# HIITMetagenomics/dsm-framework

Hardware: AMD Instinct MI355X
Metric: enumerated substrings/sec (Emax=2.0) (higher is better)
Workload: dtype u32

## Files before the change

### dsm-framework_amd/csrc/engine.hip

```cpp
#include <sched.h>

#include <algorithm>
#include <atomic>
#include <chrono>
#include <cmath>
#include <condition_variable>
#include <cstdlib>
#include <cstring>
#include <deque>
#include <map>
#include <functional>
#include <memory>
#include <mutex>
#include <sstream>
#include <thread>
#include <type_traits>

#include "common.h"
#include "scan.h"
#include "setorder.h"
#include "stream_parse.h"
#include "lfstep.h"
#include "entropy_tables.h"
#include "textemit.h"
// ... 134 lines not shown
        for (u32 l = 0; l < x.nlocal; ++l) {
            const u32 m = pb[(u64)l * x.F + u];
#pragma unroll
            for (int c = 0; c < 4; ++c) nT4[c] += (m >> c) & 1u;
        }
    }
}

template <typename P>
__global__ __launch_bounds__(256) void advance_reduce_kernel(Xchg x, u16* __restrict__ sinfo, u64* __restrict__ kplane, u32* __restrict__ cnt4, u32 nbp) {
    __shared__ u32 wtot[4][4];
    const u32 u = blockIdx.x * TILE + threadIdx.x;
    const int lane = threadIdx.x & 63, w = threadIdx.x >> 6;
    u32 nT4[4] = {0, 0, 0, 0};
    if (u < x.F) {
        parent_eval<P>(x, u, nT4);
        uint2 q;
        q.x = nT4[0] | (nT4[1] << 16);
        q.y = nT4[2] | (nT4[3] << 16);
        *reinterpret_cast<uint2*>(sinfo + (size_t)u * 4) = q;
    }
    u64 bal[4];
#pragma unroll
    for (int c = 0; c < 4; ++c) bal[c] = __ballot(nT4[c] != 0);
    if (lane < 4) {
        const u64 b = DSM_PICK(bal, lane);
        wtot[w][lane] = (u32)__popcll(b);
        kplane[((size_t)blockIdx.x * 4 + w) * 4 + lane] = b;
    }
    __syncthreads();
    if (threadIdx.x < 4) cnt4[(size_t)threadIdx.x * nbp + blockIdx.x] = wtot[0][threadIdx.x] + wtot[1][threadIdx.x] + wtot[2][threadIdx.x] + wtot[3][threadIdx.x];
}

struct FilterArgs {
    u32 F;
    u32 depth;
    u32 d;
    u32 pmin, pmax, mindepth;
    double emin, emax;
    u32 exact_order;
};

constexpr double ENT_MARGIN = 1e-4;

template <typename P>
__device__ __forceinline__ bool filter_node(const FilterArgs& a, const Xchg& x, u32 v, u32 t, u32 nc, u32 same) {
    if (a.depth < a.mindepth) return false;
    if (a.pmax != 0 && t > a.pmax) return false;
    if (t < a.pmin) return false;
    if (nc == 1 && same) return false;
    u64 sumN = a.d;
    double s = 0;
    u32 l = 0xFF;
    if (x_is_nm8(x)) {
        u32 w[8];
        x_words8(x, v, w);
#pragma unroll
        for (int g = 0; g < 8; ++g) {
            const u64 f = w[g] & (PACK_FMAX - 1);
            if (f) {
                const u32 lg = w[g] >> 13;
                l = l == 0xFF ? lg : (l == lg ? l : 5u);
                sumN += f;
                if (a.emax > 0) s += (double)(f + 1) * (double)__log2f((float)(f + 1));
            }
        }
    } else {
        for (u32 g = 0; g < a.d; ++g) {
            u64 f = (u64)x_freq<P>(x, g, v);
            if (f) {
                u32 lg = x_pl<P>(x, g, v) >> 4;
                l = l == 0xFF ? lg : (l == lg ? l : 5u);
                sumN += f;
                if (a.emax > 0) s += (double)(f + 1) * (double)__log2f((float)(f + 1));
            }
        }
    }
    if (l >= 1 && l <= 4) return false;
    if (a.emax > 0) {
        double e = (double)__log2f((float)sumN) - s / (double)sumN;
        if (e < a.emin - ENT_MARGIN || e > a.emax + ENT_MARGIN) return false;
    }
    return true;
}

constexpr u32 PW_CHUNK = 16;
constexpr u32 SREC_FIRST = 4u, SREC_LAST = 8u;
__device__ __forceinline__ uint2 child_path_word(const uint2 parent, u32 u, u32 plevel, u32 c) {
    const u32 r = plevel & (PW_CHUNK - 1);
    return r == 0 ? make_uint2(u, c) : make_uint2(parent.x, parent.y | (c << (2 * r)));
}

struct AdvanceOut {
    u32* slot;
    uint2* sa;
    uint2* pw;
    const uint2* parent_pw;
    const u32* width;
    u32 pw_after_slot;
    u32 plevel;
    u32 kshift;
    u32 cand_copy;
    u16* nT;
    u8* samechild;
    const u16* parent_nT;
    const u64* kplane;
    u64* kplane_w;
    u32* kcum;
    const u32* cnt4;
    u32* cnt_clear;
    u32 nbp;
    const u16* sinfo;
    u32 eval;
    u32 single;
    u32* const* rp;
    u32* rp0;
    const u64* const* splane;
    u32 rp_index;
    const u32* const* tpos;
    u32 nlocal, rank;
    u32 seg;
    u32 cap;
    u32* h_totals;
    u32 filter_on;
    FilterArgs fa;
    u64* candbits;
    u64* wsum;
    uint4* crec;
    u32 crec_cap;
};

struct PublishArgs {
    const u32* total;
    const u64* cand;
    const u8* cmax_base;
    u64 cmax_bpr;
    u32 cmax_world;
    u32* clear;
    u32* next;
    uint4* packet;
    u32 seq;
    uint4* bc_header;
    const u32* grand;
};
__global__ void publish_kernel(PublishArgs a) {
    __shared__ u32 wide;
    if (threadIdx.x == 0) wide = 0;
    __syncthreads();
    for (u32 r = threadIdx.x; r < a.cmax_world; r += blockDim.x) {
        const u64 m = *reinterpret_cast<const u64*>(a.cmax_base + (u64)r * a.cmax_bpr);
        if (m >= PACK_FMAX) atomicOr(&wide, m >= 65535 ? 3u : 2u);
    }
    const u32 tot = threadIdx.x == 0 ? *a.total : 0u;
    u64 cand = threadIdx.x == 0 && a.cand ? *a.cand : 0ull;
    if (threadIdx.x == 0 && a.grand) { const u64 c = (u64)(*a.grand - tot); cand = c | (c << 32); }
    __syncthreads();
    if (a.clear && threadIdx.x < 4) a.clear[threadIdx.x] = 0;
    if (threadIdx.x == 0) {
        if (a.next) { a.next[0] = tot; a.next[1] = wide; }
        const uint4 pk = make_uint4(a.seq, tot | ((wide & 1u) << 31) | ((wide >> 1) << 30), (u32)cand, (u32)(cand >> 32));
        if (a.bc_header) *a.bc_header = make_uint4(BC_OK, pk.y, 0u, 0u);
        *a.packet = pk;
    }
}

template <typename P>
// ... 97 lines not shown
        }
    }
    if (threadIdx.x == 0) o.h_totals[0] = total;
}

template <typename P>
__global__ __launch_bounds__(256) void advance_wave_kernel(Xchg x, AdvanceOut o) {
    __shared__ u32 wcnt[4][4];
    const u32 F = (u32)x.F;
    const int lane = threadIdx.x & 63;
    const u32 nw = (F + 63) >> 6;
    const u32 tile = xcd_block();
    const u32 wi = (u32)__builtin_amdgcn_readfirstlane((int)(threadIdx.x >> 6));
    const u32 w = tile * 4 + wi;
    const bool wave_in = w < nw;
    const u32 wc = wave_in ? w : 0u;
    const u64 lt = (1ull << lane) - 1;
    const u32 u = w * 64 + lane;
    const bool in = wave_in && u < F;
    const u32 uc = in ? u : 0u;
    u64 up[4];
    u32 base[4];
#pragma unroll
    for (int c = 0; c < 4; ++c) {
        up[c] = o.kplane[((size_t)wc << o.kshift) + c];
        base[c] = o.cnt4[(size_t)c * o.nbp + tile];
    }
    uint2 mypw = make_uint2(0u, 0u);
    uint2* pw = o.pw;
    u32 width = 0;
    if (o.pw_after_slot) width = o.width[0];
    if (pw) mypw = o.parent_pw[uc];
    uint2 sq = make_uint2(0u, 0u);
    if (o.sinfo) sq = *reinterpret_cast<const uint2*>(o.sinfo + (size_t)uc * 4);
    u32 myT = 1u;
    if (!o.single) myT = (u32)o.parent_nT[uc];
    u64 candw = 0;
    if (o.cand_copy && (lane == 4 || lane == 5)) candw = o.kplane[((size_t)wc << 3) + lane];
    u64 f1 = 0;
    u32 l1 = 0;
    if (o.single && o.filter_on) { f1 = (u64)x_freq<P>(x, 0, uc); l1 = x_pl<P>(x, 0, uc) >> 4; }
    if (!wave_in) {
#pragma unroll
        for (int c = 0; c < 4; ++c) up[c] = 0;
    }
    if (lane < 4) wcnt[wi][lane] = (u32)__popcll(DSM_PICK(up, lane));
    __syncthreads();
    if (!wave_in) return;
    if (o.pw_after_slot) pw = reinterpret_cast<uint2*>(reinterpret_cast<u8*>(o.slot) + (((size_t)width * 4 + 255) & ~(size_t)255));
    u32 cum[4];
#pragma unroll
    for (int c = 0; c < 4; ++c) {
        u32 before = 0;
#pragma unroll
        for (u32 q = 0; q < 3; ++q) before += q < wi ? wcnt[q][c] : 0u;
        cum[c] = base[c] + before;
    }
    u32 nT4[4] = {0, 0, 0, 0};
    if (o.sinfo) {
        if (in) { nT4[0] = sq.x & 0xFFFFu; nT4[1] = sq.x >> 16; nT4[2] = sq.y & 0xFFFFu; nT4[3] = sq.y >> 16; }
    } else {
#pragma unroll
        for (int c = 0; c < 4; ++c) nT4[c] = (u32)((up[c] >> lane) & 1);
    }
    if (lane < 4) {
        o.kcum[(size_t)w * 4 + lane] = DSM_PICK(cum, lane);
        if (o.kplane_w) o.kplane_w[(size_t)w * 4 + lane] = DSM_PICK(up, lane);
        if (o.cnt_clear && wi == 0) o.cnt_clear[(size_t)lane * o.nbp + tile] = 0;
    }
    if (o.cand_copy) {
        if (lane == 4) o.candbits[w] = candw;
        if (lane == 5) o.wsum[w] = candw;
    }
    u32 pres = 0, lastT = 0, vj[4];
#pragma unroll
    for (int c = 0; c < 4; ++c) {
        vj[c] = cum[c] + (u32)__popcll(up[c] & lt);
        if (nT4[c]) { pres |= 1u << c; lastT = nT4[c]; }
    }
    const u32 nc = __popc(pres);
    if (!in) myT = 0;
    const u32 same = o.single ? 1u : ((nc == 1 && lastT == myT) ? 1u : 0u);
    if (o.filter_on) {
        bool cand;
        if (o.single) {
            const FilterArgs& a = o.fa;
            cand = in && a.depth >= a.mindepth && 1u >= a.pmin && nc != 1 && !(f1 != 0 && l1 >= 1 && l1 <= 4);
            if (cand && a.emax > 0) {
                const u64 sumN = 1ull + f1;
                const double sl = f1 ? (double)(f1 + 1) * (double)__log2f((float)(f1 + 1)) : 0.0;
                const double e = (double)__log2f((float)sumN) - sl / (double)sumN;
                if (e < a.emin - ENT_MARGIN || e > a.emax + ENT_MARGIN) cand = false;
            }
        } else {
            cand = in && filter_node<P>(o.fa, x, u, myT, nc, same);
        }
        const u64 bits = __ballot(cand);
        u64 pairs = (u64)__popcll(bits);
        if (!o.single) pairs = wave_sum_u64(cand ? (u64)myT : 0ull);
        if (lane == 0) { o.candbits[w] = bits; o.wsum[w] = (u64)__popcll(bits) | (pairs << 32); }
    }
    if (!in) return;
    if (!o.single) o.samechild[u] = (u8)same;
#pragma unroll
    for (int c = 0; c < 4; ++c) {
        if (((pres >> c) & 1u) && vj[c] < o.cap) {
            if (o.slot) o.slot[vj[c]] = 4u * u + (u32)c;
            if (pw) pw[vj[c]] = child_path_word(mypw, u, o.plevel, (u32)c);
            if (o.sa) o.sa[vj[c]] = make_uint2(u, (u32)c | ((pres & ((1u << c) - 1u)) ? 0u : SREC_FIRST) | ((pres >> (c + 1)) ? 0u : SREC_LAST));
            if (!o.single) o.nT[vj[c]] = (u16)nT4[c];
        }
    }
    if (o.single) {
#pragma unroll
        for (int c = 0; c < 4; ++c)
            if (((pres >> c) & 1u) && vj[c] < o.cap) o.rp0[vj[c]] = (u32)c * o.seg + w * 64u + (u32)__popcll(up[c] & lt);
        return;
    }
    for (u32 sl = 0; sl < o.nlocal && pres && (o.tpos || o.rp_index); ++sl) {
        u32* rp = o.rp[sl];
        if (o.tpos) {
            const u32 m = x_pl<P>(x, o.rank * o.nlocal + sl, u) & 15u;
            const u32 h = m ? o.tpos[sl][u] : 0u;
#pragma unroll
            for (int c = 0; c < 4; ++c)
                if (((pres >> c) & 1u) && vj[c] < o.cap) rp[vj[c]] = ((m >> c) & 1u) ? h + (u32)__popc(m & ((1u << c) - 1u)) : DEAD;
        } else {
            const u64* sp = o.splane[sl] + (size_t)w * 4;
#pragma unroll
            for (int c = 0; c < 4; ++c) {
                if (!((pres >> c) & 1u) || vj[c] >= o.cap) continue;
                const u64 mine = sp[c];
                rp[vj[c]] = ((mine >> lane) & 1) ? (u32)c * o.seg + w * 64u + (u32)__popcll(mine & lt) : DEAD;
            }
        }
    }
}

template <typename P>
__global__ __launch_bounds__(256) void advance_single_kernel(Xchg x, AdvanceOut o) {
    const int lane = threadIdx.x & 63;
    const u32 F = (u32)x.F;
    const u32 nw = (F + 63) >> 6;
    const u32 tile = (u32)__builtin_amdgcn_readfirstlane((int)(xcd_block() * 4 + (threadIdx.x >> 6)));
    if (tile >= o.nbp) return;
    const u64 lt = (1ull << lane) - 1;
    const u64* __restrict__ line = o.kplane + (size_t)tile * 32;
    uint2 mypw[4];
#pragma unroll
    for (int q = 0; q < 4; ++q) {
        const u32 u = (tile * 4 + (u32)q) * 64 + lane;
        mypw[q] = o.parent_pw[u < F ? u : 0u];
    }
    u64 copyw = 0;
    if (lane < 32) copyw = line[lane];
    u32 cum[4];
#pragma unroll
    for (int c = 0; c < 4; ++c) cum[c] = o.cnt4[(size_t)c * o.nbp + tile];
    u64 up[4][4];
#pragma unroll
    for (int q = 0; q < 4; ++q)
#pragma unroll
        for (int c = 0; c < 4; ++c) up[q][c] = tile * 4 + (u32)q < nw ? line[q * 8 + c] : 0ull;
    {
        const u32 q = (u32)lane >> 3, j = (u32)lane & 7u, w = tile * 4 + q;
        if (lane < 32 && w < nw) {
            if (j < 4) o.kplane_w[(size_t)w * 4 + j] = copyw;
            else if (o.cand_copy && j == 4) o.candbits[w] = copyw;
            else if (o.cand_copy && j == 5) o.wsum[w] = copyw;
        }
    }
    const u32 r = o.plevel & (PW_CHUNK - 1);
    u32 kc = 0;
    u32 cbase = 0;
    u64 cbq[4] = {0, 0, 0, 0};
    u32 ncq[4] = {0, 0, 0, 0};
    u64 fq[4] = {0, 0, 0, 0};
    if (o.crec) {
        cbase = o.cnt4[(size_t)4 * o.nbp + tile] - o.cnt4[(size_t)4 * o.nbp];
#pragma unroll
        for (int q = 0; q < 4; ++q) {
            if (tile * 4 + (u32)q < nw) { cbq[q] = line[q * 8 + 4]; ncq[q] = (u32)line[q * 8 + 5]; }
            const u32 u = (tile * 4 + (u32)q) * 64 + lane;
            if ((cbq[q] >> lane) & 1ull) fq[q] = (u64)x_freq<P>(x, 0, u);
        }
    }
#pragma unroll
    for (int q = 0; q < 4; ++q) {
        const u32 w = tile * 4 + (u32)q, u = w * 64 + lane;
        const uint2 ppw = mypw[q];
        if (o.crec && cbq[q]) {
            const u32 k = cbase + bits_below_lane(cbq[q]);
            if (((cbq[q] >> lane) & 1ull) && k < o.crec_cap) o.crec[k] = make_uint4(u, 0u, (u32)fq[q], (u32)(fq[q] >> 32));
        }
        cbase += ncq[q];
#pragma unroll
        for (int c = 0; c < 4; ++c) {
            const u64 m = up[q][c];
            if (lane == q * 4 + c) kc = cum[c];
            const u32 below = bits_below_lane(m);
            const u32 vj = cum[c] + below;
            if (((m >> lane) & 1ull) && vj < o.cap) {
                o.rp0[vj] = (u32)c * o.seg + w * 64u + below;
                o.pw[vj] = r == 0 ? make_uint2(u, (u32)c) : make_uint2(ppw.x, ppw.y | ((u32)c << (2 * r)));
            }
            cum[c] += (u32)__popcll(m);
        }
    }
    if (lane < 16 && tile * 4 + ((u32)lane >> 2) < nw) o.kcum[(size_t)tile * 16 + lane] = kc;
}

__global__ __launch_bounds__(256) void lite_count_kernel(const u64* __restrict__ kplane, u32 nw, u32* __restrict__ cnt4, u32 nbp, u32 kshift, u32 cand_row = 0) {
    const u32 tile = blockIdx.x * 64 + (threadIdx.x >> 2), c = threadIdx.x & 3;
    if (tile >= nbp) return;
    u32 s = 0, nc = 0;
    if (cand_row && tile * 4 + c < nw) nc = (u32)kplane[((size_t)(tile * 4 + c) << 3) + 5];
#pragma unroll
    for (u32 q = 0; q < 4; ++q) {
        const u32 w = tile * 4 + q;
        if (w < nw) s += (u32)__popcll(kplane[((size_t)w << kshift) + c]);
    }
    cnt4[(size_t)c * nbp + tile] = s;
    if (cand_row) {
        nc += __shfl_xor(nc, 1, 64);
        nc += __shfl_xor(nc, 2, 64);
        if (c == 0) cnt4[(size_t)4 * nbp + tile] = nc;
    }
}
__global__ __launch_bounds__(256) void lite_slot_kernel(const u64* __restrict__ kplane, u32 F, const u32* __restrict__ cnt4, u32 nbp, u32 single_tile,
                                                        u32* __restrict__ slot, u32 cap) {
    const int lane = threadIdx.x & 63;
    const u32 nw = (F + 63) >> 6;
    const u32 tile = xcd_block();
    const u32 wi = threadIdx.x >> 6, w = tile * 4 + wi;
    if (w >= nw) return;
    const u32 u = w * 64 + lane;
    u32 base = 0;
#pragma unroll
    for (int c = 0; c < 4; ++c) {
        u32 before = 0, all = 0;
#pragma unroll
        for (u32 q = 0; q < 4; ++q) {
            const u32 wq = tile * 4 + q;
            const u32 t = wq < nw ? (u32)__popcll(kplane[(size_t)wq * 4 + c]) : 0u;
            before += q < wi ? t : 0u;
            all += t;
        }
        const u64 up = kplane[(size_t)w * 4 + c];
        const u32 first = (single_tile ? base : cnt4[(size_t)c * nbp + tile]) + before;
        base += all;
        const u32 vj = first + (u32)__popcll(up & ((1ull << lane) - 1));
        if (u < F && ((up >> lane) & 1) && vj < cap) slot[vj] = 4u * u + (u32)c;
    }
}

template <typename P>
__global__ __launch_bounds__(256) void order_kernel(u32 F, Xchg x, const u16* __restrict__ nT, const u64* __restrict__ order, Kids kids,
                                                    u64* __restrict__ order_next) {
    __shared__ u32 qn;
    __shared__ u32 qu[256];
    __shared__ u64 qm[256], qo[256];
    if (threadIdx.x == 0) qn = 0;
    __syncthreads();
    const u32 u = blockIdx.x * blockDim.x + threadIdx.x;
    if (u < F) {
        const u32 cnt = nT[u];
        const u64 ord = order[u];
        u64 mbyid = 0;
        u32 um = 0;
        if (x_is_nm8(x)) {
            u32 w[8];
            x_words8(x, u, w);
#pragma unroll
            for (int g = 0; g < 8; ++g) { const u32 m = (w[g] >> 9) & 15u; mbyid |= (u64)m << (4 * g); um |= m; }
        } else {
            for (u32 k = 0; k < cnt; ++k) {
                const u32 r = (u32)((ord >> (4 * k)) & 15);
                const u32 m = x_pl<P>(x, r, u) & 15u;
                mbyid |= (u64)m << (4 * r);
                um |= m;
            }
        }
        if (um && !(um & (um - 1))) {
            u64 rev = 0;
            for (u32 k = 0; k < cnt; ++k) {
                const u32 r = (u32)((ord >> (4 * k)) & 15);
                if ((mbyid >> (4 * r)) & 15) rev = (rev << 4) | r;
            }
            order_next[kid_index(kids, u, (u32)(__ffs((int)um) - 1))] = rev;
        } else if (um) {
            const u32 q = atomicAdd(&qn, 1u);
            qu[q] = u; qm[q] = mbyid; qo[q] = ord;
// ... 1474 lines not shown
        x.nm = node_major(w9) ? 1u : 0u;
        return x;
    }

    int alloc_kids(LevelHost& lv) {
        const size_t nw = ((size_t)lv.n + TILE - 1) / TILE * 4;
        ARENA_GET(lv.kplane, u64, 4 * nw);
        ARENA_GET(lv.kcum, u32, 4 * nw);
        return 0;
    }

    hipEvent_t pool_event(size_t k) {
        while (evpool.size() <= k) {
            hipEvent_t e = nullptr;
            if (hipEventCreateWithFlags(&e, hipEventDisableSystemFence) != hipSuccess) return nullptr;
            evpool.push_back(e);
        }
        return evpool[k];
    }

    struct BcastGuard {
        Engine* e;
        size_t gather_bytes = 0;
        void* gather_into = nullptr;
        size_t bytes = 0;
        explicit BcastGuard(Engine* e_) : e(e_) {}
        void arm(size_t b) { gather_bytes = 0; bytes = b; }
        void arm_next(size_t g, void* into, size_t b) { gather_bytes = g; gather_into = into; bytes = b; }
        void disarm() { gather_bytes = 0; bytes = 0; }
        ~BcastGuard() {
            if (!bytes) return;
            if (gather_bytes) (void)e->prm.gather(e->prm.owner_ctx, e->owner, e->xsend, gather_into, gather_bytes, (void*)e->st);
            const u32 hdr[4] = {BC_ABORT, 0, 0, 0};
            if (hipMemcpyAsync(e->bc_buf, hdr, 16, hipMemcpyHostToDevice, e->st) == hipSuccess) (void)hipStreamSynchronize(e->st);
            (void)e->prm.bcast(e->prm.owner_ctx, e->owner, e->bc_buf, bytes, (void*)e->st);
        }
    };

    u32 col_bytes(bool w16, bool w9) const { return w9 ? 2u : (w16 ? 3u : (u32)sizeof(P) + 1); }
    u64 level_bytes(u32 F, bool w16, bool w9) const { return (((u64)nlocal * F * col_bytes(w16, w9) + 15) & ~15ull) + 16; }
    static size_t bcast_bytes(u32 F) { return 16 + (size_t)((F + 63) >> 6) * 32; }
    u32 level_cap(bool w16) const { return w16 ? Fcap : FcapW; }
    int check_width(u32 Fn, bool w16) {
        if (Fn > level_cap(w16)) return fail(DSM_E_CAPACITY, "frontier wider than the device buffers: use a longer prefix or a larger arena_bytes");
        return 0;
    }
    u32 decode_level(u32 word, bool* w16, bool* w9) const {
        *w16 = !(word >> 31) && !trie_mode;
        *w9 = *w16 && !((word >> 30) & 1u);
        return word & 0x3FFFFFFFu;
    }
    int upload_order(int k, const u16* ro, size_t n) {
        if (d <= 13) {
            u64 ord = 0;
            for (size_t i = 0; i < n; ++i) ord |= (u64)ro[i] << (4 * i);
            DSM_HIP(hipMemcpyAsync(order[k], &ord, sizeof(u64), hipMemcpyHostToDevice, st));
        } else {
            DSM_HIP(hipMemcpyAsync(order16[k], ro, n * sizeof(u16), hipMemcpyHostToDevice, st));
        }
        return 0;
    }

    struct Walk {
        std::string prefix;
        RunOpts o;
        std::vector<LevelHost> L;
        u32 order_mode = 0;
        bool emitting = false;
        bool emit_failed = false;
        bool trace = false;
        size_t nev = 0;
        u32 F = 1, depth = 0;
        bool w16 = false, w9 = false;
        BcastGuard owed;
        explicit Walk(Engine* e) : owed(e) {}
        int cur() const { return (int)(depth & 1); }
    };
    struct Sweep {
        Xchg x;
        size_t mark = 0;
        u32* slot = nullptr;
        bool filtered = false;
        u32 crec_cap = 0;
        u32 Fn = 0;
        bool w16 = false, w9 = false;
        bool spec_hit = false;
    };

    int run(const char* prefix_c, dsm_tuple_sink tsink, dsm_byte_sink bsink, void* ctx, const RunOpts& o = RunOpts()) {
        Walk w(this);
        w.prefix = prefix_c ? prefix_c : "";
        w.o = o;
        for (char ch : w.prefix)
            if (ch != 'A' && ch != 'C' && ch != 'G' && ch != 'T')
                return fail(DSM_E_INVAL, "prefix must be over A,C,G,T");
        DSM_HIP(hipSetDevice(device));
        for (int s_ = 0; s_ < nlocal && !trie_mode; ++s_)
            if (!idx[s_]->dev.blk) return fail(DSM_E_INVAL, "an index of this miner is offloaded: dsm_index_reload first");
        arena.off = 0;
        earena.off = 0;
        carena.off = 0;
        w.emitting = o.emit;
        w.L.reserve(512);
        DSM_HIP(hipMemsetAsync(d_counters, 0, (size_t)COUNTER_SHARDS * 8 * sizeof(u64), st));
        if (cntraw) DSM_HIP(hipMemsetAsync(cntraw, 0, (4 * (size_t)(Seg / TILE) + 8) * sizeof(u32), st));
        DSM_HIP(hipEventRecord(ev0, st));
        if (int rc = root_level(w)) return rc;
        w.order_mode = (d < 2 || prm.pmax == 1) ? 0u : (d <= 13 ? 1u : 2u);
        stats.pair_order_exact = 1;
        w.trace = getenv("DSM_TRACE_LEVELS") != nullptr;
        DSM_HIP(hipMemsetAsync(multi ? xsend : xrecv[0], 0, XHDR, st));
        if (int rc = launch_lf(w, 0, 1, w.w16, w.w9, w.L[0].slot)) return rc;
        while (true) {
            if (int rc = exchange(w)) return rc;
            if (owner_mode && !is_owner) {
                bool more = false;
                if (int rc = client_level(w, &more)) return rc;
                if (!more) break;
                continue;
            }
            if (owner_mode) { if (int rc = owner_precheck(w)) return rc; }
            Sweep s;
            LevelHost child;
            if (int rc = advance(w, s)) return rc;
            if (int rc = publish(w, s)) return rc;
            if (int rc = commit(w, s, child)) return rc;
            if (int rc = capture_level(w, s.Fn, child.slot, child.pw)) return rc;
            if (s.filtered) {
                int erc = emit_store(w.L[w.depth], w.F, w.depth, s.x, w.cur(), w.order_mode, s.crec_cap);
                if (erc == DSM_E_CAPACITY && multi) { w.emit_failed = true; w.emitting = false; }
                else if (erc) return erc;
            }
            DSM_HIP(hipGetLastError());
            if (pend.submit && (w.F >= 200000u || w.depth >= 24)) { if (int rc = flush_pending()) return rc; }
            count_level(w);
            if (!s.Fn) break;
            w.L.push_back(child);
            step(w, s.Fn, s.w16, s.w9);
            if (w.L.size() > 60000) return fail(DSM_E_CAPACITY, "trie deeper than 60000 levels");
        }
        timeline("levels done", w.prefix.c_str());
        if (int rc = flush_pending()) return rc;
        if (int rc = finish_prefix(w, tsink, bsink, ctx)) return rc;
        return read_back(w);
    }

    int root_level(Walk& w) {
        const char* bases = "ACGT";
        for (int s = 0; s < nlocal && trie_mode; ++s) {
            const u32 zero = 0;
            DSM_HIP(hipMemcpyAsync(rp[0][s], &zero, sizeof(u32), hipMemcpyHostToDevice, st));
            stats.reported += tries[s]->nodes;
        }
        for (int s = 0; s < nlocal && !trie_mode; ++s) {
            const IndexMeta& m = idx[s]->meta;
            P h[REC_FIELDS];
            for (int f = 0; f < REC_FIELDS; ++f) h[f] = 0;
            h[0] = 0;
            h[1] = (P)(m.n - 1);
            u8 hmask = 0;
            int slot = 0;
            for (int a = 0; a < 4; ++a) {
                u64 lo = m.C[(int)bases[a]], cnt = m.codes[(int)bases[a]].count;
                if (cnt) { h[2 + 2 * slot] = (P)lo; h[3 + 2 * slot] = (P)(lo + cnt - 1); ++slot; hmask |= (u8)(1u << a); }
            }
            for (int f = 0; f < REC_FIELDS; ++f)
                DSM_HIP(hipMemcpyAsync(rec[0][s] + (size_t)f * RcapW, &h[f], sizeof(P), hipMemcpyHostToDevice, st));
            DSM_HIP(hipMemcpyAsync(rec[0][s] + (size_t)REC_FIELDS * RcapW, &hmask, 1, hipMemcpyHostToDevice, st));
            const u32 zero = 0;
            DSM_HIP(hipMemcpyAsync(rp[0][s], &zero, sizeof(u32), hipMemcpyHostToDevice, st));
            if (self_mode) {
                const u64 one = 1;
                DSM_HIP(hipMemcpyAsync(splane2[s], &one, sizeof(u64), hipMemcpyHostToDevice, st));
            }
            stats.lf_steps += 8;
            for (int a = 0; a < 4; ++a) stats.rank_ops += 2 * m.lfcost[a];
        }
        LevelHost root;
        root.n = 1;
        ARENA_GET(root.slot, u32, 1);
        ARENA_GET(root.pw, uint2, 1);
        if (int rc = alloc_kids(root)) return rc;
        if (self_mode) DSM_HIP(hipMemsetAsync(root.slot, 0, sizeof(u32), st));
        DSM_HIP(hipMemsetAsync(root.pw, 0, sizeof(uint2), st));
        w.L.push_back(root);
        u16 rootT = (u16)d;
        DSM_HIP(hipMemcpyAsync(nT[0], &rootT, sizeof(u16), hipMemcpyHostToDevice, st));
        std::vector<u16> seq(d), ro(d + 1), tmp(so_work_size(d, d));
        for (u32 k = 0; k < d; ++k) seq[k] = (u16)k;
        set_iteration_order<u16>(seq.data(), d, ro.data(), tmp.data(), d);
        return upload_order(0, ro.data(), d);
    }

    int launch_lf(Walk& w, u32 depth, u32 F, bool w16, bool w9, const u32* lslot, u64 Fmax = 0) {
        const char* bases = "ACGT";
        const bool dynamic = Fmax != 0;
        const bool fmt_in = depth > 0 && w.w16 && !trie_mode;
        const int cur = (int)(depth & 1), nxt = cur ^ 1;
        const u32 colb = col_bytes(w16, w9), fb = colb - 1;
        u8* send = multi ? xsend : xrecv[cur];
        ExpandArgs ea;
        memset(&ea, 0, sizeof ea);
        ea.F = F; ea.nbp = (F + TILE - 1) / TILE; ea.fmin = prm.fmin; ea.w16 = w9 ? 2u : (w16 ? 1u : 0u);
        ea.seg = seg_of(w16 && !trie_mode); ea.cap = 4 * ea.seg;
        ea.seg_in = seg_of(fmt_in); ea.cap_in = 4 * ea.seg_in;
        const bool nm = node_major(w9);
        ea.cstride = nm ? (u32)nlocal : 1u;
        if (dynamic) {
            ea.dyn = d_dyn;
            ea.dyn_mask = 3u;
            ea.dyn_expect = (w16 ? 0u : 1u) | (w9 ? 0u : 2u);
            ea.fcap = level_cap(w16);
        }
        unsigned long long* d_childmax = reinterpret_cast<unsigned long long*>(send);
        if (depth < w.prefix.size()) {
            const char* q = strchr(bases, w.prefix[depth]);
            ea.allowed = 1u << (q - bases);
            ea.symbol_phase = 0;
// ... 131 lines not shown
        if (nbp > 1) {
            hipLaunchKernelGGL(lite_count_kernel, dim3((nbp + 63) / 64), dim3(256), 0, st, planes, nwv, cnt4, nbp, 2u);
            exclusive_scan<u32, u32>(cnt4, cnt4, (size_t)4 * nbp, scan_tmp, d_totals, st);
        }
        hipLaunchKernelGGL(lite_slot_kernel, dim3(nbp), dim3(256), 0, st, planes, F, cnt4, nbp, nbp == 1 ? 1u : 0u, lite_slot[nxt], Fcap);
        DSM_HIP(hipGetLastError());
        if (int rc = capture_level(w, Fn, lite_slot[nxt], nullptr)) return rc;
        if (int rc = launch_lf(w, w.depth + 1, Fn, w16, w9, lite_slot[nxt])) return rc;
        step(w, Fn, w16, w9);
        return 0;
    }

    int owner_precheck(Walk& w) {
        static const int test_owner_fail = getenv("DSM_TEST_OWNER_FAIL") ? atoi(getenv("DSM_TEST_OWNER_FAIL")) : -1;
        const size_t bc_bytes = bcast_bytes(w.F);
        w.owed.arm(bc_bytes);
        if (test_owner_fail >= 0 && (int)w.depth == test_owner_fail) return fail(DSM_E_SINK, "injected owner failure (DSM_TEST_OWNER_FAIL)");
        const size_t wc = (size_t)w.F * 4 < Fcap ? (size_t)w.F * 4 : Fcap;
        const size_t need = wc * 12 + 512 + ((wc + TILE - 1) / TILE * 4) * 48 + 4096;
        if (arena.off + need <= arena.cap) return 0;
        const u32 hdr[4] = {BC_CAPACITY, 0, 0, 0};
        DSM_HIP(hipMemcpyAsync(bc_buf, hdr, 16, hipMemcpyHostToDevice, st));
        DSM_HIP(hipStreamSynchronize(st));
        w.owed.disarm();
        if (prm.bcast(prm.owner_ctx, owner, bc_buf, bc_bytes, (void*)st)) return fail(DSM_E_SINK, "bcast callback failed");
        return fail(DSM_E_CAPACITY, "device arena exhausted: use a longer prefix or a larger arena_bytes");
    }

    int advance(Walk& w, Sweep& s) {
        const u32 F = w.F, depth = w.depth;
        const int cur = w.cur(), nxt = cur ^ 1;
        s.x = xview(cur, F, w.w16, w.w9);
        const Xchg& x = s.x;
        LevelHost& me = w.L[depth];
        if (stream_mode && depth >= 1) {
            ARENA_GET(me.srec, uint4, F);
            ARENA_GET(me.clen, u8, F);
            hipLaunchKernelGGL((keep_kernel<P>), grid_for(F), dim3(256), 0, st, F, x, sa[cur], me.srec, me.clen);
        }
        if (!stream_mode && w.emitting && depth >= 1 && depth >= w.o.emit_lo && depth <= w.o.emit_hi) {
            int erc = emit_alloc(me, F);
            if (erc == DSM_E_CAPACITY && multi) { w.emit_failed = true; w.emitting = false; }
            else if (erc) return erc;
            else s.filtered = true;
        }
        s.mark = arena.off;
        const bool keep_slot = self_mode, keep_pw = !stream_mode;
        const size_t wcap = (size_t)F * 4 < Fcap ? (size_t)F * 4 : Fcap;
        u8* window = arena.get<u8>(wcap * ((keep_slot ? 4 : 0) + (keep_pw ? 8 : 0)) + 512);
        if (!window) return fail(DSM_E_CAPACITY, "device arena exhausted: use a longer prefix or a larger arena_bytes");
        s.slot = keep_slot ? reinterpret_cast<u32*>(window) : nullptr;
        const u32 nbp = (F + TILE - 1) / TILE;
        AdvanceOut ao;
        memset(&ao, 0, sizeof ao);
        ao.slot = s.slot; ao.nT = nT[nxt]; ao.samechild = samechild;
        if (stream_mode) ao.sa = sa[nxt];
        if (keep_pw) {
            ao.pw = reinterpret_cast<uint2*>(window);
            ao.pw_after_slot = keep_slot ? 1u : 0u;
            ao.parent_pw = me.pw;
            ao.plevel = depth;
        }
        ao.parent_nT = nT[cur]; ao.nlocal = (u32)nlocal; ao.rank = (u32)rank;
        ao.cap = (u32)wcap;
        ao.seg = seg_of(w.w16 && !trie_mode);
        ao.h_totals = d_pub_tot;
        ao.rp = d_rp_tab[nxt];
        ao.rp0 = rp[nxt][0];
        ao.tpos = trie_mode ? d_tpos_tab : nullptr;
        ao.splane = d_splane_tab;
        ao.rp_index = self_mode ? 0u : 1u;
        ao.kcum = me.kcum; ao.cnt4 = cnt4; ao.nbp = nbp; ao.kshift = 2;
        ao.width = d_totals;
        const bool merged = d > 1 || trie_mode;
        if (merged && nbp == 1) {
            ao.eval = 1; ao.kplane_w = me.kplane;
        } else if (merged) {
            hipLaunchKernelGGL((advance_reduce_kernel<P>), dim3(nbp), dim3(256), 0, st, x, sinfo, me.kplane, cnt4, nbp);
            ao.kplane = me.kplane; ao.sinfo = sinfo;
        } else {
            ao.kplane = splane[0]; ao.kplane_w = me.kplane; ao.single = 1;
            ao.kshift = 3;
        }
        const bool lean = !merged && nbp > 1 && keep_pw && !keep_slot && !stream_mode;
        if (lean && s.filtered && carena.cap) {
            const size_t room = (carena.cap - carena.off) / sizeof(uint4);
            s.crec_cap = (u32)(room < (size_t)F ? room : (size_t)F);
        }
        const bool fold = s.crec_cap > 0;
        if (nbp > 1) {
            if (!merged) hipLaunchKernelGGL(lite_count_kernel, dim3((nbp + 63) / 64), dim3(256), 0, st, splane[0], (F + 63) >> 6, cntraw, nbp, 3u, fold ? 1u : 0u);
            exclusive_scan<u32, u32>(merged ? cnt4 : cntraw, cnt4, (size_t)(fold ? 5 : 4) * nbp, scan_tmp, d_totals, st);
        }
        const bool fused_filter = s.filtered && nbp > 1;
        if (fused_filter) {
            ao.fa = filter_args(F, depth, w.order_mode); ao.candbits = me.cand_bits; ao.wsum = cand_wsum;
            if (ao.single) ao.cand_copy = 1;
            else ao.filter_on = 1;
        }
        if (fold) { ao.crec = reinterpret_cast<uint4*>(carena.base + carena.off); ao.crec_cap = s.crec_cap; }
        if (nbp == 1) hipLaunchKernelGGL((advance_down_kernel<P>), dim3(1), dim3(256), 0, st, x, ao);
        else if (lean) hipLaunchKernelGGL((advance_single_kernel<P>), dim3((nbp + 3) / 4), dim3(256), 0, st, x, ao);
        else hipLaunchKernelGGL((advance_wave_kernel<P>), dim3(nbp), dim3(256), 0, st, x, ao);
        if (s.filtered) {
            if (int erc = emit_filter(me, F, depth, x, cur, w.order_mode, !fused_filter, fold)) return erc;
        }
        return 0;
    }

    int publish(Walk& w, Sweep& s) {
        const u32 F = w.F, nbp = (F + TILE - 1) / TILE;
        const int nxt = w.cur() ^ 1;
        PublishArgs pa;
        memset(&pa, 0, sizeof pa);
        pa.total = nbp == 1 ? d_pub_tot : d_totals;
        pa.cmax_base = s.x.base; pa.cmax_bpr = s.x.bpr; pa.cmax_world = (u32)world;
        if (s.filtered) pa.cand = d_totals64;
        if (s.crec_cap) {
            pa.total = cnt4 + (size_t)4 * nbp;
            pa.grand = d_totals;
            pa.cand = nullptr;
        }
        pa.clear = reinterpret_cast<u32*>(multi ? xsend : xrecv[nxt]);
        pa.packet = reinterpret_cast<uint4*>(h_totals + 304); pa.seq = ++pub_seq;
        pa.next = spec_mode ? d_dyn : nullptr;
        pa.bc_header = owner_mode ? reinterpret_cast<uint4*>(bc_buf) : nullptr;
        hipLaunchKernelGGL(publish_kernel, dim3(1), dim3(64), 0, st, pa);
        if (owner_mode) {
            const size_t bc_bytes = bcast_bytes(F);
            DSM_HIP(hipMemcpyAsync(bc_buf + 16, w.L[w.depth].kplane, bc_bytes - 16, hipMemcpyDeviceToDevice, st));
            w.owed.disarm();
            if (prm.bcast(prm.owner_ctx, owner, bc_buf, bc_bytes, (void*)st)) return fail(DSM_E_SINK, "bcast callback failed");
            stats.exchange_bytes_sent += bc_bytes * (u64)(world - 1);
        }
        if (spec_mode) { if (int rc = launch_lf(w, w.depth + 1, 0, w.w16, w.w9, s.slot, (u64)F * 4)) return rc; }
        u32 pk[4];
        if (int rc = wait_packet(pk)) return rc;
        s.Fn = decode_level(pk[1], &s.w16, &s.w9);
        s.spec_hit = spec_mode && s.Fn > 0 && s.Fn <= level_cap(s.w16) && s.w16 == w.w16 && s.w9 == w.w9;
        if (spec_mode && !s.spec_hit) --stats.expand_launches;
        h_totals[300] = pk[2]; h_totals[301] = pk[3];
        if (int rc = check_width(s.Fn, s.w16)) return rc;
        if (owner_mode) {
            if (!s.Fn) w.owed.arm(16);
            else w.owed.arm_next((size_t)level_bytes(s.Fn, s.w16, s.w9), xrecv[nxt], bcast_bytes(s.Fn));
        }
        return 0;
    }
    int wait_packet(u32 pk[4]) {
        volatile u32* fl = h_totals + 304;
        u32 spins = 0;
        while (*fl != pub_seq) {
            if ((++spins & 0xFFFFu) == 0 && hipStreamQuery(st) != hipErrorNotReady) {
                DSM_HIP(hipStreamSynchronize(st));
                if (*fl != pub_seq) return fail(DSM_E_HIP, "publish kernel did not report");
                break;
            }
            __builtin_ia32_pause();
        }
        std::atomic_thread_fence(std::memory_order_acquire);
        for (int q = 0; q < 4; ++q) pk[q] = fl[q];
        return 0;
    }

    int commit(Walk& w, const Sweep& s, LevelHost& child) {
        const u32 F = w.F, Fn = s.Fn;
        const int cur = w.cur(), nxt = cur ^ 1;
        arena.off = s.mark;
        child.n = Fn;
        if (!Fn) return 0;
        if (self_mode) child.slot = arena.get<u32>(Fn);
        if (!stream_mode) child.pw = arena.get<uint2>(Fn);
        if (int rc = alloc_kids(child)) return rc;
        if (s.spec_hit) {
            stats.expand_slots += Fn;
            stats.expand_column_bytes += (u64)Fn * col_bytes(s.w16, s.w9);
        } else {
            if (int rc = launch_lf(w, w.depth + 1, Fn, s.w16, s.w9, child.slot)) return rc;
        }
        const Kids kids = w.L[w.depth].kids();
        if (!(w.o.emit || w.o.capture)) {}
        else if (w.order_mode == 1)
            hipLaunchKernelGGL((order_kernel<P>), grid_for(F), dim3(256), 0, st, F, s.x, nT[cur], order[cur], kids, order[nxt]);
        else if (w.order_mode == 2 && d <= 64)
            hipLaunchKernelGGL((order_big_kernel<P, 64>), grid_for(F, 64), dim3(64), 0, st, F, s.x, nT[cur], order16[cur], kids, order16[nxt]);
        else if (w.order_mode == 2)
            hipLaunchKernelGGL((order_big_kernel<P, 273>), grid_for(F, 64), dim3(64), 0, st, F, s.x, nT[cur], order16[cur], kids, order16[nxt]);
        if (w.order_mode && w.o.seed && w.depth + 1 == w.o.seed->depth) {
            const std::vector<u16>& so = w.o.seed->ord[0];
            if (int rc = upload_order(nxt, so.data(), so.size())) return rc;
        }
        return 0;
    }

    int capture_level(Walk& w, u32 Fn, const u32* slot, const uint2* pw) {
        NodeOrder* cap = w.o.capture;
        if (!Fn || !cap || w.depth + 1 != cap->depth) return 0;
        const int nxt = w.cur() ^ 1;
        const bool client = owner_mode && !is_owner;
        std::vector<u32> hs(Fn);
        std::vector<u16> hn(Fn);
        if (slot) DSM_HIP(hipMemcpyAsync(hs.data(), slot, (size_t)Fn * sizeof(u32), hipMemcpyDeviceToHost, st));
        else if (stream_mode) {
            std::vector<uint2> hr(Fn);
            DSM_HIP(hipMemcpyAsync(hr.data(), sa[nxt], (size_t)Fn * sizeof(uint2), hipMemcpyDeviceToHost, st));
            DSM_HIP(hipStreamSynchronize(st));
            for (u32 v = 0; v < Fn; ++v) hs[v] = hr[v].y & 3u;
        } else {
            std::vector<uint2> hp(Fn);
            DSM_HIP(hipMemcpyAsync(hp.data(), pw, (size_t)Fn * sizeof(uint2), hipMemcpyDeviceToHost, st));
            DSM_HIP(hipStreamSynchronize(st));
            for (u32 v = 0; v < Fn; ++v) hs[v] = (hp[v].y >> (2 * (w.depth % PW_CHUNK))) & 3u;
        }
        if (!client) DSM_HIP(hipMemcpyAsync(hn.data(), nT[nxt], (size_t)Fn * sizeof(u16), hipMemcpyDeviceToHost, st));
        DSM_HIP(hipStreamSynchronize(st));
        const u32 order_mode = client ? 0u : w.order_mode;
        cap->sym.clear();
        cap->ord.clear();
        for (u32 v = 0; v < Fn; ++v) {
            cap->sym.push_back(hs[v] & 3);
            std::vector<u16> o(d == 1 || client ? 1 : hn[v]);
            if (order_mode == 1) {
                u64 ord = 0;
                DSM_HIP(hipMemcpy(&ord, order[nxt] + v, sizeof(u64), hipMemcpyDeviceToHost));
                for (u32 k = 0; k < hn[v]; ++k) o[k] = (u16)((ord >> (4 * k)) & 15);
            } else if (order_mode == 2) {
                DSM_HIP(hipMemcpy(o.data(), order16[nxt] + (size_t)v * d, (size_t)hn[v] * sizeof(u16), hipMemcpyDeviceToHost));
            }
            cap->ord.push_back(o);
        }
        return 0;
    }

    void count_level(const Walk& w) {
        if (w.trace) {
            if (owner_mode && !is_owner) fprintf(stderr, "dsm level prefix=%s depth=%u F=%u (client of rank %d)\n", w.prefix.c_str(), w.depth, w.F, owner);
            else fprintf(stderr, "dsm level prefix=%s depth=%u F=%u\n", w.prefix.c_str(), w.depth, w.F);
        }
        stats.union_nodes += w.depth >= 1 ? w.F : 0;
        if (w.F > stats.max_frontier) stats.max_frontier = w.F;
        ++stats.levels;
    }
    void step(Walk& w, u32 Fn, bool w16, bool w9) {
        w.F = Fn;
        ++w.depth;
        w.w16 = w16;
        w.w9 = w9;
    }

    int finish_prefix(Walk& w, dsm_tuple_sink tsink, dsm_byte_sink bsink, void* ctx) {
        const u32 nlev = (u32)w.L.size();
        if (stream_mode) {
            if (w.o.emit) { if (int rc = finish_stream(w.L, nlev, bsink, ctx)) return rc; }
            return 0;
        }
        bool ready = false;
        if (w.emitting) {
            int rc = finish_mine(w.L, nlev, tsink, ctx, &ready);
            if (rc == DSM_E_CAPACITY && multi) { w.emit_failed = true; ready = false; }
            else if (rc) return rc;
        }
        if (owner_mode) {
            u32 hdr[4] = {w.emit_failed ? BC_CAPACITY : BC_OK, 0, 0, 0};
            if (is_owner) {
                DSM_HIP(hipMemcpyAsync(bc_buf, hdr, 16, hipMemcpyHostToDevice, st));
                DSM_HIP(hipStreamSynchronize(st));
            }
            w.owed.disarm();
            if (prm.bcast(prm.owner_ctx, owner, bc_buf, 16, (void*)st)) return fail(DSM_E_SINK, "bcast callback failed");
            if (!is_owner) {
                DSM_HIP(hipMemcpyAsync(hdr, bc_buf, 16, hipMemcpyDeviceToHost, st));
                DSM_HIP(hipStreamSynchronize(st));
            }
            if (hdr[0] == BC_ABORT) return fail(DSM_E_SINK, "the prefix's owner failed and aborted the prefix (its own error says why)");
            if (hdr[0] != BC_OK) return fail(DSM_E_CAPACITY, "device arena exhausted on the prefix's owner: use a longer prefix or a larger arena_bytes");
        } else if (multi) {
            u64 ok = w.emit_failed ? 0 : 1, all_ok = 0;
            if (int rc = agree_min(ok, &all_ok)) return rc;
            if (!all_ok) return fail(DSM_E_CAPACITY, "device arena exhausted on a rank: use a longer prefix or a larger arena_bytes");
        }
        if (ready) pend.submit = true;
        else pend.E = nullptr;
        return 0;
    }

    int read_back(const Walk& w) {
        DSM_HIP(hipEventRecord(ev1, st));
        timeline("finish queued", w.prefix.c_str());
        DSM_HIP(hipStreamSynchronize(st));
        timeline("device done", w.prefix.c_str());
        float ms = 0;
        DSM_HIP(hipEventElapsedTime(&ms, ev0, ev1));
        stats.device_ms += ms;
        float expand_ms = 0;
        for (size_t k = 0; k + 1 < w.nev; k += 2) {
            float t = 0;
            DSM_HIP(hipEventElapsedTime(&t, evpool[k], evpool[k + 1]));
            expand_ms += t;
        }
        stats.expand_ms += expand_ms;
        u64 hc[NCOUNTERS] = {0, 0, 0, 0, 0, 0};
        {
            std::vector<u64> sh((size_t)COUNTER_SHARDS * 8);
            DSM_HIP(hipMemcpy(sh.data(), d_counters, sh.size() * sizeof(u64), hipMemcpyDeviceToHost));
            for (int k = 0; k < COUNTER_SHARDS; ++k)
                for (int c = 0; c < NCOUNTERS; ++c) hc[c] += sh[(size_t)k * 8 + c];
#ifdef DSM_CLOCK_PROBE
            if (sh[7]) {
                double dur = 0, ramp = 0, tail = 0, meanbusy = 0;
                int nl = 0;
                const double W = (double)lfgeo.blocks * lfgeo.waves_per_block;
                for (int k = 1; k + 2 < COUNTER_SHARDS; k += 3) {
                    const u64 s0 = ~sh[(size_t)k * 8 + 6], s9 = sh[(size_t)k * 8 + 7], e0 = ~sh[(size_t)(k + 1) * 8 + 6], e9 = sh[(size_t)(k + 1) * 8 + 7];
                    if (!s9 || e9 - s0 < 5000) continue;
                    const double ms = (double)sh[(size_t)(k + 2) * 8 + 6] / W, me = (double)sh[(size_t)(k + 2) * 8 + 7] / W;
                    dur += (double)(e9 - s0); ramp += (double)(s9 - s0); tail += (double)(e9 - e0); meanbusy += me - ms; ++nl;
                }
                fprintf(stderr, "clock probe: %.1f MHz; %d launches >= 50 us: duration %.2f ms, first-to-last wave start %.2f ms, first-to-last wave end %.2f ms, mean wave busy %.2f ms\n",
                        (double)sh[6] / (double)sh[7] * 100.0, nl, dur * 1e-5, ramp * 1e-5, tail * 1e-5, meanbusy * 1e-5);
            }
// ... 579 lines not shown
```

Measured before the change: 19.58 billion.

## Add fused narrow advance kernel folding count, scan, filter and publish

For frontiers up to a configurable tile count, a new advance_narrow_kernel replaces the lite_count, exclusive_scan, advance, emit_filter and publish launches with one kernel. Each block recomputes its prefix offsets by popcounting all kplane lines, and the single-tile case evaluates the entropy filter inline. Tile 0 writes the publish packet. This removes several small launches per level in exchange for redundant per-block scanning work, which grows with the number of tiles.

```diff
diff --git a/dsm-framework_amd/csrc/engine.hip b/dsm-framework_amd/csrc/engine.hip
--- a/dsm-framework_amd/csrc/engine.hip
+++ b/dsm-framework_amd/csrc/engine.hip
@@ -240,6 +240,16 @@
         if (e < a.emin - ENT_MARGIN || e > a.emax + ENT_MARGIN) return false;
     }
     return true;
+}
+__device__ __forceinline__ bool filter_single(const FilterArgs& a, u32 nc, u64 f1, u32 l1) {
+    bool cand = a.depth >= a.mindepth && 1u >= a.pmin && nc != 1 && !(f1 != 0 && l1 >= 1 && l1 <= 4);
+    if (cand && a.emax > 0) {
+        const u64 sumN = 1ull + f1;
+        const double sl = f1 ? (double)(f1 + 1) * (double)__log2f((float)(f1 + 1)) : 0.0;
+        const double e = (double)__log2f((float)sumN) - sl / (double)sumN;
+        if (e < a.emin - ENT_MARGIN || e > a.emax + ENT_MARGIN) cand = false;
+    }
+    return cand;
 }
 
 constexpr u32 PW_CHUNK = 16;
@@ -503,19 +513,7 @@
     if (!in) myT = 0;
     const u32 same = o.single ? 1u : ((nc == 1 && lastT == myT) ? 1u : 0u);
     if (o.filter_on) {
-        bool cand;
-        if (o.single) {
-            const FilterArgs& a = o.fa;
-            cand = in && a.depth >= a.mindepth && 1u >= a.pmin && nc != 1 && !(f1 != 0 && l1 >= 1 && l1 <= 4);
-            if (cand && a.emax > 0) {
-                const u64 sumN = 1ull + f1;
-                const double sl = f1 ? (double)(f1 + 1) * (double)__log2f((float)(f1 + 1)) : 0.0;
-                const double e = (double)__log2f((float)sumN) - sl / (double)sumN;
-                if (e < a.emin - ENT_MARGIN || e > a.emax + ENT_MARGIN) cand = false;
-            }
-        } else {
-            cand = in && filter_node<P>(o.fa, x, u, myT, nc, same);
-        }
+        const bool cand = in && (o.single ? filter_single(o.fa, nc, f1, l1) : filter_node<P>(o.fa, x, u, myT, nc, same));
         const u64 bits = __ballot(cand);
         u64 pairs = (u64)__popcll(bits);
         if (!o.single) pairs = wave_sum_u64(cand ? (u64)myT : 0ull);
@@ -558,14 +556,26 @@
     }
 }
 
-template <typename P>
-__global__ __launch_bounds__(256) void advance_single_kernel(Xchg x, AdvanceOut o) {
-    const int lane = threadIdx.x & 63;
+struct TileLines {
+    u64 up[4][4];
+    u64 cb[4];
+    u32 nc[4];
+};
+__device__ __forceinline__ void tile_lines(const AdvanceOut& o, u32 tile, u32 nw, TileLines& t) {
+    const u64* __restrict__ line = o.kplane + (size_t)tile * 32;
+#pragma unroll
+    for (int q = 0; q < 4; ++q) {
+        const bool in = tile * 4 + (u32)q < nw;
+#pragma unroll
+        for (int c = 0; c < 4; ++c) t.up[q][c] = in ? line[q * 8 + c] : 0ull;
+        t.cb[q] = in && o.crec ? line[q * 8 + 4] : 0ull;
+        t.nc[q] = in && o.crec ? (u32)line[q * 8 + 5] : 0u;
+    }
+}
+template <typename P, bool EVAL>
+__device__ __forceinline__ u32 single_tile_sweep(const Xchg& x, const AdvanceOut& o, u32 tile, int lane, const TileLines& t, u32 cum[4], u32 cbase) {
     const u32 F = (u32)x.F;
     const u32 nw = (F + 63) >> 6;
-    const u32 tile = (u32)__builtin_amdgcn_readfirstlane((int)(xcd_block() * 4 + (threadIdx.x >> 6)));
-    if (tile >= o.nbp) return;
-    const u64 lt = (1ull << lane) - 1;
     const u64* __restrict__ line = o.kplane + (size_t)tile * 32;
     uint2 mypw[4];
 #pragma unroll
@@ -575,14 +585,6 @@
     }
     u64 copyw = 0;
     if (lane < 32) copyw = line[lane];
-    u32 cum[4];
-#pragma unroll
-    for (int c = 0; c < 4; ++c) cum[c] = o.cnt4[(size_t)c * o.nbp + tile];
-    u64 up[4][4];
-#pragma unroll
-    for (int q = 0; q < 4; ++q)
-#pragma unroll
-        for (int c = 0; c < 4; ++c) up[q][c] = tile * 4 + (u32)q < nw ? line[q * 8 + c] : 0ull;
     {
         const u32 q = (u32)lane >> 3, j = (u32)lane & 7u, w = tile * 4 + q;
         if (lane < 32 && w < nw) {
@@ -593,16 +595,15 @@
     }
     const u32 r = o.plevel & (PW_CHUNK - 1);
     u32 kc = 0;
-    u32 cbase = 0;
     u64 cbq[4] = {0, 0, 0, 0};
     u32 ncq[4] = {0, 0, 0, 0};
     u64 fq[4] = {0, 0, 0, 0};
     if (o.crec) {
-        cbase = o.cnt4[(size_t)4 * o.nbp + tile] - o.cnt4[(size_t)4 * o.nbp];
 #pragma unroll
         for (int q = 0; q < 4; ++q) {
-            if (tile * 4 + (u32)q < nw) { cbq[q] = line[q * 8 + 4]; ncq[q] = (u32)line[q * 8 + 5]; }
-            const u32 u = (tile * 4 + (u32)q) * 64 + lane;
+            const u32 w = tile * 4 + (u32)q, u = w * 64 + lane;
+            if (EVAL) continue;
+            cbq[q] = t.cb[q]; ncq[q] = t.nc[q];
             if ((cbq[q] >> lane) & 1ull) fq[q] = (u64)x_freq<P>(x, 0, u);
         }
     }
@@ -610,6 +611,14 @@
     for (int q = 0; q < 4; ++q) {
         const u32 w = tile * 4 + (u32)q, u = w * 64 + lane;
         const uint2 ppw = mypw[q];
+        if (EVAL && o.crec && w < nw) {
+            const u32 uc = u < F ? u : 0u;
+            fq[q] = (u64)x_freq<P>(x, 0, uc);
+            const u32 nc = (u32)((t.up[q][0] >> lane) & 1) + (u32)((t.up[q][1] >> lane) & 1) + (u32)((t.up[q][2] >> lane) & 1) + (u32)((t.up[q][3] >> lane) & 1);
+            cbq[q] = __ballot(u < F && filter_single(o.fa, nc, fq[q], x_pl<P>(x, 0, uc) >> 4));
+            ncq[q] = (u32)__popcll(cbq[q]);
+            if (lane == 0) { o.candbits[w] = cbq[q]; o.wsum[w] = (u64)ncq[q] | ((u64)ncq[q] << 32); }
+        }
         if (o.crec && cbq[q]) {
             const u32 k = cbase + bits_below_lane(cbq[q]);
             if (((cbq[q] >> lane) & 1ull) && k < o.crec_cap) o.crec[k] = make_uint4(u, 0u, (u32)fq[q], (u32)(fq[q] >> 32));
@@ -617,7 +626,7 @@
         cbase += ncq[q];
 #pragma unroll
         for (int c = 0; c < 4; ++c) {
-            const u64 m = up[q][c];
+            const u64 m = t.up[q][c];
             if (lane == q * 4 + c) kc = cum[c];
             const u32 below = bits_below_lane(m);
             const u32 vj = cum[c] + below;
@@ -629,6 +638,106 @@
         }
     }
     if (lane < 16 && tile * 4 + ((u32)lane >> 2) < nw) o.kcum[(size_t)tile * 16 + lane] = kc;
+    return ncq[0] + ncq[1] + ncq[2] + ncq[3];
+}
+
+template <typename P>
+__global__ __launch_bounds__(256) void advance_single_kernel(Xchg x, AdvanceOut o) {
+    const int lane = threadIdx.x & 63;
+    const u32 tile = (u32)__builtin_amdgcn_readfirstlane((int)(xcd_block() * 4 + (threadIdx.x >> 6)));
+    if (tile >= o.nbp) return;
+    u32 cum[4];
+#pragma unroll
+    for (int c = 0; c < 4; ++c) cum[c] = o.cnt4[(size_t)c * o.nbp + tile];
+    const u32 cbase = o.crec ? o.cnt4[(size_t)4 * o.nbp + tile] - o.cnt4[(size_t)4 * o.nbp] : 0u;
+    TileLines t;
+    tile_lines(o, tile, ((u32)x.F + 63) >> 6, t);
+    single_tile_sweep<P, false>(x, o, tile, lane, t, cum, cbase);
+}
+
+template <typename P>
+__global__ __launch_bounds__(256, 8) void advance_narrow_kernel(Xchg x, AdvanceOut o, PublishArgs a) {
+    __shared__ u64 part[4][5];
+    __shared__ u32 own[4][5];
+    const int lane = threadIdx.x & 63;
+    const u32 nw = ((u32)x.F + 63) >> 6;
+    const u32 group = xcd_block();
+    const u32 wi = (u32)__builtin_amdgcn_readfirstlane((int)(threadIdx.x >> 6));
+    const u32 tile = group * 4 + wi;
+    u32 cum[4] = {0, 0, 0, 0}, all[4], cbase = 0, call = 0;
+    TileLines t;
+    tile_lines(o, tile, tile < o.nbp ? nw : 0u, t);
+    if (o.nbp > 1) {
+        u64 acc[5] = {0, 0, 0, 0, 0};
+        const u32 first = group * 16;
+#pragma unroll 2
+        for (u32 i = threadIdx.x; i < nw; i += 256) {
+            const u64* __restrict__ ln = o.kplane + (size_t)i * 8;
+            const u64 keep = i < first ? ~0ull : ~0ull << 32;
+            u64 n[5];
+#pragma unroll
+            for (int c = 0; c < 4; ++c) n[c] = (u64)__popcll(ln[c]);
+            n[4] = ln[5] & 0xFFFFFFFFull;
+#pragma unroll
+            for (int k = 0; k < 5; ++k) acc[k] += (n[k] | (n[k] << 32)) & keep;
+        }
+        u32 mine[5] = {0, 0, 0, 0, 0};
+#pragma unroll
+        for (int q = 0; q < 4; ++q) {
+#pragma unroll
+            for (int c = 0; c < 4; ++c) mine[c] += (u32)__popcll(t.up[q][c]);
+            mine[4] += t.nc[q];
+        }
+#pragma unroll
+        for (int k = 0; k < 5; ++k) {
+            const u64 s = wave_sum_u64(acc[k]);
+            if (lane == 0) { part[wi][k] = s; own[wi][k] = mine[k]; }
+        }
+        __syncthreads();
+        if (tile >= o.nbp) return;
+        u32 before[5];
+#pragma unroll
+        for (int k = 0; k < 5; ++k) {
+            const u64 s = part[0][k] + part[1][k] + part[2][k] + part[3][k];
+            u32 b = (u32)s;
+#pragma unroll
+            for (u32 q = 0; q < 3; ++q) b += q < wi ? own[q][k] : 0u;
+            before[k] = (u32)__builtin_amdgcn_readfirstlane((int)b);
+            if (k < 4) all[k] = (u32)__builtin_amdgcn_readfirstlane((int)(u32)(s >> 32));
+            else call = (u32)__builtin_amdgcn_readfirstlane((int)(u32)(s >> 32));
+        }
+        u32 lower = 0;
+#pragma unroll
+        for (int c = 0; c < 4; ++c) { cum[c] = lower + before[c]; lower += all[c]; }
+        cbase = before[4];
+        single_tile_sweep<P, false>(x, o, tile, lane, t, cum, cbase);
+    } else {
+        if (wi != 0) return;
+#pragma unroll
+        for (int c = 0; c < 4; ++c) {
+            all[c] = 0;
+#pragma unroll
+            for (int q = 0; q < 4; ++q) all[c] += (u32)__popcll(t.up[q][c]);
+        }
+        u32 lower = 0;
+#pragma unroll
+        for (int c = 0; c < 4; ++c) { cum[c] = lower; lower += all[c]; }
+        call = o.filter_on ? single_tile_sweep<P, true>(x, o, 0u, lane, t, cum, 0u) : single_tile_sweep<P, false>(x, o, 0u, lane, t, cum, 0u);
+    }
+    if (tile != 0) return;
+    u32 wide = 0;
+    for (u32 rk = (u32)lane; rk < a.cmax_world; rk += 64) {
+        const u64 m = *reinterpret_cast<const u64*>(a.cmax_base + (u64)rk * a.cmax_bpr);
+        if (m >= PACK_FMAX) wide |= m >= 65535 ? 3u : 2u;
+    }
+    wide = (__ballot(wide & 1u) ? 1u : 0u) | (__ballot(wide & 2u) ? 2u : 0u);
+    const u32 tot = all[0] + all[1] + all[2] + all[3];
+    const u32 cand = o.crec ? call : 0u;
+    if (a.clear && lane < 4) a.clear[lane] = 0;
+    if (lane == 0) {
+        if (a.next) { a.next[0] = tot; a.next[1] = wide; }
+        *a.packet = make_uint4(a.seq, tot | ((wide & 1u) << 31) | ((wide >> 1) << 30), cand, cand);
+    }
 }
 
 __global__ __launch_bounds__(256) void lite_count_kernel(const u64* __restrict__ kplane, u32 nw, u32* __restrict__ cnt4, u32 nbp, u32 kshift, u32 cand_row = 0) {
@@ -2269,6 +2378,8 @@
         u32* slot = nullptr;
         bool filtered = false;
         u32 crec_cap = 0;
+        bool narrow = false;
+        const char* sweep = "";
         u32 Fn = 0;
         bool w16 = false, w9 = false;
         bool spec_hit = false;
@@ -2320,7 +2431,7 @@
             }
             DSM_HIP(hipGetLastError());
             if (pend.submit && (w.F >= 200000u || w.depth >= 24)) { if (int rc = flush_pending()) return rc; }
-            count_level(w);
+            count_level(w, &s);
             if (!s.Fn) break;
             w.L.push_back(child);
             step(w, s.Fn, s.w16, s.w9);
@@ -2618,34 +2729,44 @@
             ao.kplane = splane[0]; ao.kplane_w = me.kplane; ao.single = 1;
             ao.kshift = 3;
         }
-        const bool lean = !merged && nbp > 1 && keep_pw && !keep_slot && !stream_mode;
-        if (lean && s.filtered && carena.cap) {
+        const bool mined1 = !merged && keep_pw && !keep_slot && !stream_mode;
+        const bool lean = mined1 && nbp > 1;
+        const bool few = mined1 && nbp <= narrow_tiles() && !multi && !owner_mode && prm.pmin <= 1;
+        if ((lean || few) && s.filtered && carena.cap) {
             const size_t room = (carena.cap - carena.off) / sizeof(uint4);
             s.crec_cap = (u32)(room < (size_t)F ? room : (size_t)F);
         }
         const bool fold = s.crec_cap > 0;
-        if (nbp > 1) {
+        s.narrow = few && (!s.filtered || fold);
+        if (nbp > 1 && !s.narrow) {
             if (!merged) hipLaunchKernelGGL(lite_count_kernel, dim3((nbp + 63) / 64), dim3(256), 0, st, splane[0], (F + 63) >> 6, cntraw, nbp, 3u, fold ? 1u : 0u);
             exclusive_scan<u32, u32>(merged ? cnt4 : cntraw, cnt4, (size_t)(fold ? 5 : 4) * nbp, scan_tmp, d_totals, st);
         }
-        const bool fused_filter = s.filtered && nbp > 1;
+        const bool fused_filter = s.filtered && (nbp > 1 || s.narrow);
         if (fused_filter) {
             ao.fa = filter_args(F, depth, w.order_mode); ao.candbits = me.cand_bits; ao.wsum = cand_wsum;
-            if (ao.single) ao.cand_copy = 1;
+            if (ao.single && nbp > 1) ao.cand_copy = 1;
             else ao.filter_on = 1;
         }
         if (fold) { ao.crec = reinterpret_cast<uint4*>(carena.base + carena.off); ao.crec_cap = s.crec_cap; }
-        if (nbp == 1) hipLaunchKernelGGL((advance_down_kernel<P>), dim3(1), dim3(256), 0, st, x, ao);
+        if (s.narrow) hipLaunchKernelGGL((advance_narrow_kernel<P>), dim3((nbp + 3) / 4), dim3(256), 0, st, x, ao, publish_args(w, s));
+        else if (nbp == 1) hipLaunchKernelGGL((advance_down_kernel<P>), dim3(1), dim3(256), 0, st, x, ao);
         else if (lean) hipLaunchKernelGGL((advance_single_kernel<P>), dim3((nbp + 3) / 4), dim3(256), 0, st, x, ao);
         else hipLaunchKernelGGL((advance_wave_kernel<P>), dim3(nbp), dim3(256), 0, st, x, ao);
-        if (s.filtered) {
+        s.sweep = s.narrow ? "narrow" : (nbp == 1 ? "down" : (lean ? "single" : "wave"));
+        if (s.filtered && !s.narrow) {
             if (int erc = emit_filter(me, F, depth, x, cur, w.order_mode, !fused_filter, fold)) return erc;
         }
         return 0;
     }
 
-    int publish(Walk& w, Sweep& s) {
-        const u32 F = w.F, nbp = (F + TILE - 1) / TILE;
+    static u32 narrow_tiles() {
+        static const u32 v = [] { const char* e = getenv("DSM_NARROW_TILES"); return e ? (u32)atol(e) : 1024u; }();
+        return v;
+    }
+
+    PublishArgs publish_args(const Walk& w, const Sweep& s) {
+        const u32 nbp = (w.F + TILE - 1) / TILE;
         const int nxt = w.cur() ^ 1;
         PublishArgs pa;
         memset(&pa, 0, sizeof pa);
@@ -2661,7 +2782,13 @@
         pa.packet = reinterpret_cast<uint4*>(h_totals + 304); pa.seq = ++pub_seq;
         pa.next = spec_mode ? d_dyn : nullptr;
         pa.bc_header = owner_mode ? reinterpret_cast<uint4*>(bc_buf) : nullptr;
-        hipLaunchKernelGGL(publish_kernel, dim3(1), dim3(64), 0, st, pa);
+        return pa;
+    }
+
+    int publish(Walk& w, Sweep& s) {
+        const u32 F = w.F;
+        const int nxt = w.cur() ^ 1;
+        if (!s.narrow) hipLaunchKernelGGL(publish_kernel, dim3(1), dim3(64), 0, st, publish_args(w, s));
         if (owner_mode) {
             const size_t bc_bytes = bcast_bytes(F);
             DSM_HIP(hipMemcpyAsync(bc_buf + 16, w.L[w.depth].kplane, bc_bytes - 16, hipMemcpyDeviceToDevice, st));
@@ -2768,10 +2895,12 @@
         return 0;
     }
 
-    void count_level(const Walk& w) {
+    void count_level(const Walk& w, const Sweep* s = nullptr) {
         if (w.trace) {
             if (owner_mode && !is_owner) fprintf(stderr, "dsm level prefix=%s depth=%u F=%u (client of rank %d)\n", w.prefix.c_str(), w.depth, w.F, owner);
-            else fprintf(stderr, "dsm level prefix=%s depth=%u F=%u\n", w.prefix.c_str(), w.depth, w.F);
+            else
+                fprintf(stderr, "dsm level prefix=%s depth=%u F=%u sweep=%s cand=%u block=%u\n", w.prefix.c_str(), w.depth, w.F, s ? s->sweep : "",
+                        w.L[w.depth].ncand, s ? s->crec_cap : 0u);
         }
         stats.union_nodes += w.depth >= 1 ? w.F : 0;
         if (w.F > stats.max_frontier) stats.max_frontier = w.F;
```

Measured after the change: 19.77 billion, median of 6. About the same (+1.0%).
